# AgentCooper2002/AudioDiffuser

Hardware: AMD Instinct MI355X
Metric: audio samples/sec (16384-sample waveform, 50-step Heun) (higher is better)
Workload: dtype bf16; 1 GPU; BASELINE configs[1]: UNet1d 64 ch (c2), 16384-sample waveforms, KarrasSchedule N=50 heun, batch 64/GPU, random-init weights; global_batch=64, sampler=heun, num_steps=50, nfe=99, hipgraph=True, parallelism=batch-sharded x1, one all-gather

## Files before the change

audiodiffuser_amd/_lib.py:

```python
from __future__ import annotations

import ctypes as C
import os
from typing import Optional

from .config import UNet1dConfig

HERE = os.path.dirname(os.path.abspath(__file__))
LIB_PATH = os.environ.get("ADF_HIP_LIB") or os.path.join(HERE, "libadf_hip.so")
ADF_MAX_LAYERS = 12
DTYPE_F32, DTYPE_BF16, DTYPE_F32X3 = 0, 1, 2
FLAG_SEPARATE_GN_STATS = 1
SAMPLER_EDM, SAMPLER_EDM_ALPHA, SAMPLER_DPM_MULTISTEP, SAMPLER_DPM2, SAMPLER_ADPM2 = 0, 1, 2, 3, 4
SAMPLER_LMS, SAMPLER_DPM_SINGLESTEP, SAMPLER_DPM2M, SAMPLER_UNIPC, SAMPLER_ADPMPP2S = 5, 6, 7, 8, 9
SAMPLER_RF_EULER = 10


class AdfNetConfig(C.Structure):
    _fields_ = [
        ("channels", C.c_int32), ("num_filters", C.c_int32), ("window_length", C.c_int32), ("stride", C.c_int32),
        ("in_channels", C.c_int32), ("out_channels", C.c_int32),
        ("resnet_groups", C.c_int32), ("kernel_multiplier_downsample", C.c_int32),
        ("num_layers", C.c_int32),
        ("multipliers", C.c_int32 * (ADF_MAX_LAYERS + 1)),
# ... 116 lines not shown
    "adf_unet2d_create": (C.c_int, [C.POINTER(AdfUNet2dConfig), C.POINTER(C.c_void_p)]),
    "adf_dit_create": (C.c_int, [C.POINTER(AdfDitConfig), C.POINTER(C.c_void_p)]),
    "adf_set_image_shape": (C.c_int, [C.c_void_p, C.c_int, C.c_int]),
    "adf_set_dynamic_threshold": (C.c_int, [C.c_void_p, C.c_float]),
    "adf_set_preconditioning": (C.c_int, [C.c_void_p, C.c_int, C.c_double, C.c_double, C.c_double]),
    "adf_debug_coef_rows": (C.c_int, [C.c_void_p, C.c_void_p, C.c_int, C.POINTER(C.c_int), C.c_void_p]),
    "adf_destroy": (None, [C.c_void_p]),
    "adf_last_error": (C.c_char_p, [C.c_void_p]),
    "adf_num_weights": (C.c_int, [C.c_void_p]),
    "adf_weight_name": (C.c_char_p, [C.c_void_p, C.c_int]),
    "adf_weight_numel": (C.c_int64, [C.c_void_p, C.c_int]),
    "adf_load_weight": (C.c_int, [C.c_void_p, C.c_char_p, C.c_void_p, C.c_int64, C.c_void_p]),
    "adf_weights_missing": (C.c_int, [C.c_void_p]),
    "adf_set_condition": (C.c_int, [C.c_void_p, C.c_void_p, C.c_int, C.c_int, C.c_float, C.c_void_p]),
    "adf_net_forward": (C.c_int, [C.c_void_p, C.c_void_p, C.c_void_p, C.c_void_p, C.c_int, C.c_int, C.c_void_p]),
    "adf_denoise": (C.c_int, [C.c_void_p, C.c_void_p, C.c_void_p, C.c_float, C.c_float, C.c_void_p, C.c_int, C.c_int, C.c_void_p]),
    "adf_sampler_run": (C.c_int, [C.c_void_p, C.POINTER(AdfSamplerDesc), C.POINTER(C.c_float), C.c_int, C.c_void_p,
                                  C.c_void_p, C.c_int, C.c_void_p, C.c_int, C.c_int, C.c_void_p]),
    "adf_diffusion_loss": (C.c_int, [C.c_void_p, C.c_int, C.c_void_p, C.c_void_p, C.c_void_p, C.c_float, C.c_void_p, C.c_void_p, C.c_void_p,
                                     C.c_int, C.c_int, C.c_void_p]),
    "adf_loss_calls": (C.c_int64, [C.c_void_p]),
    "adf_sampler_nfe": (C.c_int, [C.POINTER(AdfSamplerDesc), C.POINTER(C.c_float), C.c_int]),
    "adf_sampler_run_table": (C.c_int, [C.c_void_p, C.POINTER(AdfTableDesc), C.POINTER(AdfTableStep), C.c_void_p, C.c_void_p, C.c_int, C.c_void_p,
                                        C.c_int, C.c_int, C.c_void_p]),
    "adf_sampler_table_nfe": (C.c_int, [C.POINTER(AdfTableDesc), C.POINTER(AdfTableStep)]),
    "adf_sampler_run_program": (C.c_int, [C.c_void_p, C.POINTER(AdfProgDesc), C.POINTER(AdfProgOp), C.c_void_p, C.c_void_p, C.c_int, C.c_int, C.c_void_p]),
    "adf_sampler_program_nfe": (C.c_int, [C.POINTER(AdfProgDesc), C.POINTER(AdfProgOp)]),
    "adf_debug_tap_shape": (C.c_int, [C.c_void_p, C.c_char_p, C.POINTER(C.c_int), C.POINTER(C.c_int)]),
    "adf_debug_tap_copy": (C.c_int, [C.c_void_p, C.c_char_p, C.c_void_p, C.c_void_p]),
    "adf_debug_tap_stats": (C.c_int, [C.c_void_p, C.c_char_p, C.c_void_p, C.POINTER(C.c_int), C.c_void_p]),
    "adf_debug_rb_block_plan": (C.c_int, [C.c_int] * 9 + [C.POINTER(C.c_int)] * 5),
    "adf_debug_up_tile_plan": (C.c_int, [C.c_int, C.c_int, C.c_int, C.c_int, C.c_int, C.POINTER(C.c_int), C.POINTER(C.c_int), C.POINTER(C.c_int),
                                         C.POINTER(C.c_int)]),
    "adf_debug_dyn_threshold": (C.c_int, [C.c_void_p, C.c_void_p, C.c_int, C.c_longlong, C.c_float, C.c_void_p]),
    "adf_debug_tap_count": (C.c_int, [C.c_void_p]),
    "adf_debug_tap_name": (C.c_char_p, [C.c_void_p, C.c_int]),
    "adf_device_bytes": (C.c_int64, [C.c_void_p]),
    "adf_bench_resblock": (C.c_int, [C.c_void_p, C.c_int, C.c_int, C.c_int, C.c_int, C.POINTER(C.c_float), C.POINTER(C.c_float),
                                     C.POINTER(C.c_double), C.POINTER(C.c_double), C.POINTER(C.c_double), C.POINTER(C.c_double),
                                     C.c_void_p]),
    "adf_bench_layer": (C.c_int, [C.c_void_p, C.c_int, C.c_int, C.c_int, C.c_int, C.c_int, C.POINTER(C.c_float), C.POINTER(C.c_double),
                                  C.POINTER(C.c_double), C.POINTER(C.c_int), C.c_void_p]),
    "adf_bench_wavenet_layer": (C.c_int, [C.c_void_p, C.c_int, C.c_int, C.c_int, C.c_int, C.POINTER(C.c_float), C.POINTER(C.c_double),
                                          C.POINTER(C.c_double), C.c_void_p]),
    "adf_bench_loss_kernels": (C.c_int, [C.c_void_p, C.c_int, C.c_int, C.c_longlong, C.c_int, C.POINTER(C.c_float), C.POINTER(C.c_float),
                                         C.POINTER(C.c_double), C.POINTER(C.c_double), C.c_void_p]),
    "adf_istft_create": (C.c_int, [C.POINTER(AdfIstftConfig), C.c_void_p, C.POINTER(C.c_void_p)]),
    "adf_istft_basis": (C.c_int, [C.POINTER(AdfIstftConfig), C.c_void_p, C.c_void_p, C.c_void_p]),
    "adf_istft_run": (C.c_int, [C.c_void_p, C.c_void_p, C.c_int, C.c_int, C.c_void_p, C.c_int64, C.c_void_p]),
    "adf_istft_destroy": (None, [C.c_void_p]),
    "adf_stft_create": (C.c_int, [C.POINTER(AdfIstftConfig), C.c_void_p, C.POINTER(C.c_void_p)]),
    "adf_stft_basis": (C.c_int, [C.POINTER(AdfIstftConfig), C.c_void_p, C.c_void_p]),
    "adf_stft_run": (C.c_int, [C.c_void_p, C.c_void_p, C.c_int, C.c_int64, C.c_void_p, C.c_int, C.c_void_p]),
    "adf_stft_destroy": (None, [C.c_void_p]),
}

_lib: Optional[C.CDLL] = None


def load_library() -> C.CDLL:
    global _lib
    if _lib is not None:
        return _lib
    if not os.path.exists(LIB_PATH):
        raise RuntimeError(
            f"{LIB_PATH} is missing: build it with `python -m audiodiffuser_amd.build` "
# ... 109 lines not shown
```

audiodiffuser_amd/csrc/adf_gemm.hip:

```cpp
#include "adf_gemm.h"
#include "adf_gemm_pp.h"
#include "adf_gemm_rb.h"
#include "adf_gemm_rbx3.h"
#include "adf_gemm_up.h"
#include "adf_kernels.h"
#include <cstdio>
#include <cstdlib>
#include <cstring>
#include <vector>


#ifdef ADF_RB_STAMP
namespace adf { __device__ unsigned long long adf_rb_stamps[8 * 16]; }
extern "C" int adf_debug_rb_stamps(unsigned long long* out) {
    return (int)hipMemcpyFromSymbol(out, HIP_SYMBOL(adf::adf_rb_stamps), sizeof(unsigned long long) * 8 * 16);
}
#endif

#ifdef ADF_RB_TL
namespace adf { __device__ unsigned adf_rb_tl[2 * 8 * 128]; }
extern "C" int adf_debug_rb_timeline(unsigned* out) {
    return (int)hipMemcpyFromSymbol(out, HIP_SYMBOL(adf::adf_rb_tl), sizeof(unsigned) * 2 * 8 * 128);
}
#endif
// ... 237 lines not shown
    if (a.n != a.n_pad || a.out_c != a.n || a.n_pad % kPpTN || a.n_pad > kPpMaxN) return false;
    if (!pow2(a.mrows / tm)) return false;
    if (a.res && a.nseg > 1) return false;
    int nb = a.res ? a.n / 64 : 0;
    for (int s = 0; s < a.nseg; ++s) {
        const GemmSeg& g = a.seg[s];
        if (g.stride != 1 || g.step != 1) return false;
        if (!((g.taps == 3 && g.off0 == -1) || (g.taps == 1 && g.off0 == 0))) return false;
        if (g.c0 % 64 || g.c1 % 64 || (g.ab && g.c0 + g.c1 > kPpMaxCin)) return false;
        if (s == 1 && (g.ab || g.act)) return false;
        nb += (g.c0 + g.c1) / 64;
    }
    return nb >= 2;
}

const void* pp_identity(int n, hipStream_t stream, const char** err) {
    static void* cache_dev[kMaxDevices][kPpMaxN / 64 + 1] = {};
    void** cache = cache_dev[current_device()];
    const int idx = n / 64;
    if (cache[idx]) return cache[idx];
    const size_t elems = (size_t)(n / 64 + kTapGroup) * n * 64;
    std::vector<uint16_t> hbuf(elems, 0);
    for (int r = 0; r < n; ++r) hbuf[((size_t)(r / 64) * n + r) * 64 + (r % 64)] = 0x3F80;
    void* d = nullptr;
    if (hipMalloc(&d, elems * 2) != hipSuccess) { *err = "conv_gemm_pp: hipMalloc(identity) failed"; return nullptr; }
    if (hipMemcpyAsync(d, hbuf.data(), elems * 2, hipMemcpyHostToDevice, stream) != hipSuccess || hipStreamSynchronize(stream) != hipSuccess) {
        *err = "conv_gemm_pp: identity upload failed";
        return nullptr;
    }
    cache[idx] = d;
    return d;
}

template <typename T, int MT, int NT>
const char* launch_ksplit(const GemmArgs& a, hipStream_t stream) {
    constexpr int lds = 4 * ks_wave_lds(MT, NT);
    constexpr int TM = 32 * MT, TN = 32 * NT;
    if (!raise_lds_limit<lds, conv_gemm_ksplit_kernel<T, MT, NT>>()) return "hipFuncSetAttribute(MaxDynamicSharedMemorySize, ksplit) failed";
    const int tiles_n = (a.n_pad + TN - 1) / TN;
    const long long tiles_m = a.flat ? ((long long)a.B * a.mrows + TM - 1) / TM : (long long)((a.mrows + TM - 1) / TM) * a.B;
    const long long blocks = tiles_m * tiles_n;
    if (blocks <= 0 || blocks > 0x7fffffffLL) return "conv_gemm_ksplit: bad grid";
    hipLaunchKernelGGL((conv_gemm_ksplit_kernel<T, MT, NT>), dim3((unsigned)blocks), dim3(256), lds, stream, a);
    return hipGetLastError() == hipSuccess ? nullptr : "conv_gemm_ksplit: launch failed";
}

template <typename T>
const char* dispatch(const GemmArgs& a, int tm, int tn, hipStream_t s) {
    if (tm == 128 && tn == 128) return launch_variant<T, 2, 2, 2, 2>(a, s);
    if (tm == 128 && tn == 64) return launch_variant<T, 2, 1, 2, 2>(a, s);
    if (tm == 128 && tn == 32) return launch_variant<T, 1, 1, 4, 1>(a, s);
    if (tm == 64 && tn == 128) return launch_variant<T, 1, 2, 2, 2>(a, s);
    if (tm == 64 && tn == 64) return launch_variant<T, 1, 1, 2, 2>(a, s);
    if (tm == 64 && tn == 32) return launch_variant<T, 1, 1, 2, 1>(a, s);
    if (tm == 32 && tn == 128) return launch_variant<T, 1, 1, 1, 4>(a, s);
    if (tm == 32 && tn == 64) return launch_variant<T, 1, 1, 1, 2>(a, s);
    return launch_variant<T, 1, 1, 1, 1>(a, s);
}

struct GemmSwitches {
    int trace = adf_route_switch("ADF_GEMM_TRACE", 0);
    int up = adf_route_switch("ADF_GEMM_UP", 1);
    int pp = adf_route_switch("ADF_GEMM_PP", 1);
    int ws = adf_route_switch("ADF_GEMM_WS", 1);
    long long rb_min_tiles = min_tiles_of(adf_route_switch("ADF_GEMM_RB", 1));
    long long rbx3_min_tiles = min_tiles_of(adf_route_switch("ADF_GEMM_RBX3", 1));
    int rb_zskip = adf_route_switch("ADF_RB_ZSKIP", 1);
    int gn_in_kernel = (int)adf_tuning("ADF_GEMM_GN", 1);
    int min_blocks = (int)adf_tuning("ADF_GEMM_MINBLOCKS", 512);
    int ksplit = (int)adf_tuning("ADF_GEMM_KSPLIT", 1);
    long long ksplit_rows = adf_tuning("ADF_GEMM_KSPLIT_ROWS", 4096);
    int ksplit_minit = (int)adf_tuning("ADF_GEMM_KSPLIT_MINIT", 4);
    long long ws_min_m = adf_tuning("ADF_GEMM_WS_MINM", 256);
    static long long min_tiles_of(int sw) { return sw == 0 ? -1 : (sw >= 2 ? 32 : 256); }
};
const GemmSwitches& switches() {
    static const GemmSwitches s;
    return s;
}

enum class Route { refused, up, ksplit, rbx3, rb, pp, ws, plain };
const char* const kRouteName[] = {"", "up", "ksplit", "rbx3", "rb", "pp", "ws", "plain"};

struct GemmPlan {
    Route route = Route::refused;
    const char* refusal = nullptr;
    int tm = 0, tn = 0;
    int flat = 0, seg_rows = 0;
    bool stats = false;
    bool stats_traced = false;
    bool gn_in_kernel = false;
    int up_cfg = 0;
    bool ident_seg = false;
};

bool rb_takes(const GemmArgs& a, bool x3, bool with_stats) {
    const long long min_tiles = x3 ? switches().rbx3_min_tiles : switches().rb_min_tiles;
    const RbForm& f = x3 ? kRbX3 : kRbBf16;
    RbTiles t;
    return min_tiles >= 0 && rb_shape_ok(a, f, with_stats) && rb_tiles(a, f, min_tiles, t);
// ... 163 lines not shown
    if (!p.stats) a.stats = nullptr;
    if (a.nseg > 1) a.seg[1].gn.gamma = nullptr;
    if (p.ident_seg) {
        const char* err = nullptr;
        const void* ident = pp_identity(a.n, stream, &err);
        if (!ident) return err;
        GemmSeg& g = a.seg[1];
        g = GemmSeg{};
        g.src0 = a.res; g.src1 = nullptr; g.c0 = a.n; g.c1 = 0; g.ab = nullptr; g.scale1 = 1.0f; g.act = 0;
        g.taps = 1; g.stride = 1; g.off0 = 0; g.step = 1; g.w = ident; g.nchunk = a.n / 64;
        a.nseg = 2;
        a.res = nullptr;
    }
    if (a.seg[0].gn.gamma && !p.gn_in_kernel) {
        const char* err = a.gn_ready ? nullptr : launch_gn_finalize(a.seg[0].gn, stream);
        a.seg[0].gn.gamma = nullptr;
        if (err) return err;
    }
    if (sw.trace) {
        fprintf(stderr, "[adf gemm] %-6s B=%d lin=%d mrows=%d n=%d/%d nseg=%d seg0(c=%d+%d taps=%d stride=%d off0=%d step=%d ab=%d act=%d)", kRouteName[(int)p.route], a.B,
                a.lin, a.mrows, a.n, a.n_pad, a.nseg, a.seg[0].c0, a.seg[0].c1, a.seg[0].taps, a.seg[0].stride, a.seg[0].off0, a.seg[0].step, a.seg[0].ab != nullptr,
                a.seg[0].act);
        if (a.nseg > 1) fprintf(stderr, " seg1(c=%d+%d taps=%d ab=%d)", a.seg[1].c0, a.seg[1].c1, a.seg[1].taps, a.seg[1].ab != nullptr);
        fprintf(stderr, " res=%d gelu=%d scatter=%d out=%dx%d stats=%d flat=%d tile=%dx%d\n", a.res != nullptr, a.gelu, a.scatter_f, a.out_rows, a.out_c, p.stats_traced,
                a.flat, p.tm, p.tn);
    }
    switch (p.route) {
    case Route::up:
        if (p.up_cfg == 1) return launch_up<256, 256, 4>(a, stream);
        if (p.up_cfg == 2) return launch_up<256, 128, 2>(a, stream);
        if (p.up_cfg == 3) return launch_up<128, 128, 2>(a, stream);
        return launch_up<128, 64, 2>(a, stream);
    case Route::ksplit:
        if (p.tm == 64) return dtype == 1 ? launch_ksplit<bf16_t, 2, 2>(a, stream) : (dtype == 2 ? launch_ksplit<f32x3_t, 2, 2>(a, stream) : launch_ksplit<float, 2, 2>(a, stream));
        return dtype == 1 ? launch_ksplit<bf16_t, 1, 1>(a, stream) : (dtype == 2 ? launch_ksplit<f32x3_t, 1, 1>(a, stream) : launch_ksplit<float, 1, 1>(a, stream));
    case Route::rbx3: return launch_rbx3(a, sw.rbx3_min_tiles, stream);
    case Route::rb: return launch_rb(a, sw.rb_min_tiles, sw.rb_zskip, stream);
    case Route::pp: return p.tm == 256 ? launch_pp<2>(a, stream) : launch_pp<1>(a, stream);
    case Route::ws:
        if (p.tn == 128) return dtype == 1 ? launch_ws_variant<bf16_t, 2, 2>(a, stream) : launch_ws_variant<float, 2, 2>(a, stream);
        return dtype == 1 ? launch_ws_variant<bf16_t, 1, 2>(a, stream) : launch_ws_variant<float, 1, 2>(a, stream);
    default: return dtype == 1 ? dispatch<bf16_t>(a, p.tm, p.tn, stream) : (dtype == 2 ? dispatch<f32x3_t>(a, p.tm, p.tn, stream) : dispatch<float>(a, p.tm, p.tn, stream));
    }
}

}

extern "C" int adf_debug_rb_block_plan(int K, int f, int C, int phase_c, int n, int B, int L, int min_tiles, int zskip, int* tile_rows, int* nh, int* nb3, int* nb2,
                                       int* phase2) {
    using namespace adf;
    if (B < 1 || L < 1 || C < 1 || f < 1 || (long long)B * L > 0x3fffffffLL) return 1;
    static const char dummy[16] = {};
    GemmArgs a;
    memset(&a, 0, sizeof(a));
    a.nseg = 1; a.B = B; a.lin = a.mrows = a.out_rows = L; a.n = a.n_pad = a.out_c = a.bias_mod = n;
    a.phase_c = phase_c;
    GemmSeg& g = a.seg[0];
    g.src0 = g.w = dummy;
    g.c0 = phase_c ? C : f * C;
    g.taps = 3; g.stride = 1; g.off0 = -1; g.step = 1;
    g.tap2_zero_c = phase_c ? 0 : folded_tap2_zero_from(K, f, C);
    RbTiles t;
    if (!rb_shape_ok(a, kRbBf16, false) || !rb_tiles(a, kRbBf16, min_tiles, t)) return 1;
    RbArgs r;
    rb_fill_args(a, kRbBf16, t, zskip, r);
    if (tile_rows) *tile_rows = t.tm;
    if (nh) *nh = t.nh;
    if (nb3) *nb3 = r.h.nb3;
    if (nb2) *nb2 = r.h.nb2;
    if (phase2) *phase2 = r.h.phase2;
    return 0;
}

extern "C" int adf_debug_up_tile_plan(int cin, int cout, int f, int B, int L, int* tile_rows, int* items, int* rounds, int* dead_rows) {
    using namespace adf;
    if (B < 1 || L < 1 || (long long)B * L > 0x3fffffffLL) return 1;
    UpTilePlan tp;
    if (cin == 256 && cout == 256 && f == 4) tp = up_tile_plan(B, L, UpCfg<256, 256, 4, 1>::WROWS, UpCfg<256, 256, 4, 1>::NPASS);
    else if (cin == 256 && cout == 128 && f == 2) tp = up_tile_plan(B, L, UpCfg<256, 128, 2, 1>::WROWS, UpCfg<256, 128, 2, 1>::NPASS);
    else if (cin == 128 && cout == 128 && f == 2) tp = up_tile_plan(B, L, UpCfg<128, 128, 2, 1>::WROWS, UpCfg<128, 128, 2, 1>::NPASS);
    else if (cin == 128 && cout == 64 && f == 2) tp = up_tile_plan(B, L, UpCfg<128, 64, 2, 1>::WROWS, UpCfg<128, 64, 2, 1>::NPASS);
    else return 1;
    if (tile_rows) *tile_rows = tp.tile_rows;
    if (items) *items = (int)tp.items;
    if (rounds) *rounds = (int)tp.rounds;
    if (dead_rows) *dead_rows = tp.dead_rows;
    return 0;
}
```

audiodiffuser_amd/csrc/adf_kernels.h:

```cpp
#pragma once
#include "adf_common.h"

namespace adf {

const char* launch_gn_stats(const void* x, int bf16, int B, int L, int C, int G, double* stats, hipStream_t s);

const char* launch_gn_finalize(const GnFinalizeArgs& a, hipStream_t s);

const char* launch_gn_apply(const void* s0, const void* s1, int c0, int c1, int L, int B, const float* ab, int act, void* out,
                            int bf16, hipStream_t s);

const char* launch_gn_norm_apply(const void* s0, const void* s1, const GnFinalizeArgs& a, int act, void* out, int bf16, hipStream_t s);

const char* launch_ln_rows(const void* x, void* y, int bf16, long long rows, int C, const float* gamma,
                           const float* beta, float eps, hipStream_t s);

const char* launch_attention(const void* qkv, void* out, int bf16, int B, int N, int C, int heads, hipStream_t s);
const char* launch_attention_x3(const void* qkv, void* out, int B, int N, int C, int heads, hipStream_t s);

const char* launch_upsample_nearest_pad(const void* x, void* out, int bf16, int B, int L, int C, int f, hipStream_t s);
const char* launch_to_in(const float* x, const float* w, void* out, int bf16, int B, int in_ch, int L, int nf,
                         int wl, int stride, int pad, const float* coef, int coef_bstride, hipStream_t s);

const char* launch_to_out(const void* h, const float* w, float* out, int dtype, int B, int out_ch, int Lh, int nf,
                          int wl, int stride, int pad, int mode, const float* x_noisy, const float* coef,
                          int coef_bstride, hipStream_t s);

enum { ADF_PRECOND_KIND_EDM = 0, ADF_PRECOND_KIND_VE = 1, ADF_PRECOND_KIND_VP = 2, ADF_PRECOND_KIND_V_EDM = 3, ADF_PRECOND_KIND_RF = 4, ADF_PRECOND_KIND_RF_EDM = 5 };
struct Precond {
    int kind = ADF_PRECOND_KIND_EDM;
    float sigma_data = 1.0f;
    float beta_min2 = 0.f, two_beta_d = 0.f, beta_min = 0.f, beta_d = 1.f, m_minus_1 = 0.f;
};
const char* launch_edm_coef(const float* sigmas_dev, float sigma_scalar, int nb, const Precond& pc, float* coef,
                            hipStream_t s);
const char* launch_edm_coef_list(const float* sigmas_host, int n, const Precond& pc, float* coef, hipStream_t s);

struct TimeEmbedArgs {
    const float* t; int t_stride; int nb; int ch;
    const float* fourier; const float* w1; const float* b1; const float* w2; const float* b2;
    float* temb;
};
const char* launch_time_embed(const TimeEmbedArgs& a, hipStream_t s);

const char* launch_film(const float* in, int in_dim, const float* w, int ldw, int w_col0, const float* bias, float* film, int nb,
                        int total, hipStream_t s);
const char* launch_class_embed(const long long* classes, int num_classes, int null_all, const float* emb, const float* null_emb,
                               const float* lnw, const float* lnb, const float* w1, const float* b1, const float* w2, const float* b2,
                               int ch, int cdim, float* out, int nrows, hipStream_t s);
const char* launch_cfg_combine(float* out, const float* x, const float* fc, const float* fn, const float* coef, int coef_bstride,
                               float scale, long long per_sample, long long n, int clampit, hipStream_t s);
const char* launch_dyn_threshold(float* x, int B, long long per_sample, float q, float* scale_scratch, hipStream_t s);

const char* launch_scale(float* out, const float* in, float s, long long n, hipStream_t st);
const char* launch_churn(float* x_hat, const float* x, const float* eps, float c, float s_noise, long long n, hipStream_t st);
// ... 35 lines not shown
```

audiodiffuser_amd/csrc/adf_kernels.hip:

```cpp
#include "adf_kernels.h"

namespace adf {

#define ADF_LAUNCH_CHECK(name) (hipGetLastError() == hipSuccess ? nullptr : name ": launch failed")

template <typename T>
__global__ void __launch_bounds__(256) gn_stats_kernel(const T* __restrict__ x, int L, int C, int G, int rows_per_block,
                                                       double* __restrict__ stats) {
    constexpr int EPC = Elem<T>::kPerChunk;
    extern __shared__ __attribute__((aligned(16))) char smem[];
    float* csum = (float*)smem;
    float* csq = csum + C;
    const int b = blockIdx.y;
    const int cpr = C / EPC;
    const int tid = threadIdx.x;
    for (int i = tid; i < 2 * C; i += 256) csum[i] = 0.f;
    __syncthreads();
    const int cc = tid % cpr, rsub = tid / cpr, rstep = 256 / cpr;
    const int r0 = blockIdx.x * rows_per_block;
    const int r1 = min(L, r0 + rows_per_block);
    float s[EPC], q[EPC];
#pragma unroll
    for (int e = 0; e < EPC; ++e) { s[e] = 0.f; q[e] = 0.f; }
    const T* base = x + (size_t)b * L * C + (size_t)cc * EPC;
// ... 814 lines not shown
        const int p0 = m0 * STRIDE - 4 + i * 4;
        float4 v = {0.f, 0.f, 0.f, 0.f};
        if (p0 >= 0 && p0 + 3 < L) v = *(const float4*)(xr + p0);
        else {
            if (p0 >= 0 && p0 < L) v.x = xr[p0];
            if (p0 + 1 >= 0 && p0 + 1 < L) v.y = xr[p0 + 1];
            if (p0 + 2 >= 0 && p0 + 2 < L) v.z = xr[p0 + 2];
            if (p0 + 3 >= 0 && p0 + 3 < L) v.w = xr[p0 + 3];
        }
        *(float4*)(xs + i * 4) = float4{cin * v.x, cin * v.y, cin * v.z, cin * v.w};
    }
    float wr[WL][EPC];
#pragma unroll
    for (int k = 0; k < WL; ++k)
#pragma unroll
        for (int e = 0; e < EPC; ++e) wr[k][e] = w[(size_t)(cc * EPC + e) * WL + k];
    __syncthreads();
    const int shift = 4 - pad;
#pragma unroll 4
    for (int ml = rsub; ml < ROWS && m0 + ml < Lo; ml += rpi) {
        float acc[EPC];
#pragma unroll
        for (int e = 0; e < EPC; ++e) acc[e] = 0.f;
#pragma unroll
        for (int k = 0; k < WL; ++k) {
            const float xv = xs[ml * STRIDE + k + shift];
#pragma unroll
            for (int e = 0; e < EPC; ++e) acc[e] = fmaf(wr[k][e], xv, acc[e]);
        }
        *(u32x4_t*)(out + ((size_t)b * Lo + m0 + ml) * nf + (size_t)cc * EPC) = pack16<T>(acc);
    }
}

const char* launch_to_in(const float* x, const float* w, void* out, int bf16, int B, int in_ch, int L, int nf,
                         int wl, int stride, int pad, const float* coef, int coef_bstride, hipStream_t s) {
    const int epc = bf16 ? 8 : 4;
    if (nf % epc) return "to_in: num_filters must be a multiple of a 16-byte chunk";
    if (L % stride) return "to_in: L % stride != 0";
    const int cpr_fast = nf / epc;
    if (in_ch == 1 && wl == 8 && stride == 2 && pad >= 0 && pad <= 4 && L % 4 == 0 && cpr_fast <= 256 && (cpr_fast & (cpr_fast - 1)) == 0) {
        const int Lo = L / stride;
        dim3 grid((unsigned)((Lo + 255) / 256), B);
        if (bf16) hipLaunchKernelGGL(to_in_rows_kernel<bf16_t>, grid, dim3(256), 0, s, x, w, (bf16_t*)out, L, nf, pad, coef, coef_bstride);
        else hipLaunchKernelGGL(to_in_rows_kernel<float>, grid, dim3(256), 0, s, x, w, (float*)out, L, nf, pad, coef, coef_bstride);
        return ADF_LAUNCH_CHECK("to_in_rows");
    }
    const size_t lds = (size_t)nf * in_ch * wl * sizeof(float);
    if (lds > 60000) return "to_in: weight tile too large for LDS";
    const long long work = (long long)(L / stride) * (nf / epc);
    dim3 grid((unsigned)((work + 255) / 256), B);
    if (bf16) hipLaunchKernelGGL(to_in_kernel<bf16_t>, grid, dim3(256), lds, s, x, w, (bf16_t*)out, in_ch, L, nf, wl, stride, pad, coef, coef_bstride);
    else hipLaunchKernelGGL(to_in_kernel<float>, grid, dim3(256), lds, s, x, w, (float*)out, in_ch, L, nf, wl, stride, pad, coef, coef_bstride);
    return ADF_LAUNCH_CHECK("to_in");
}

template <typename T>
__global__ void __launch_bounds__(256) to_out_kernel(const T* __restrict__ h, const float* __restrict__ w, float* __restrict__ out,
                                                     int out_ch, int Lh, int nf, int wl, int stride, int pad, int mode,
                                                     const float* __restrict__ x_noisy, const float* __restrict__ coef,
                                                     int coef_bstride) {
    constexpr int EPC = Elem<T>::kPerChunk;
    constexpr int R = 256;
    extern __shared__ __attribute__((aligned(16))) char smem[];
    const int halo = (wl + stride - 1) / stride;
    float* ws = (float*)smem;
    float* P = ws + nf * wl;
    const int b = blockIdx.y, oc = blockIdx.z;
    for (int i = threadIdx.x; i < nf * wl; i += 256) {
        const int k = i % wl, ci = i / wl;
        ws[i] = w[((size_t)ci * out_ch + oc) * wl + k];
    }
    __syncthreads();
    const int i0 = blockIdx.x * R - halo;
    const int nrows = R + 2 * halo;
// ... 111 lines not shown
        if (r < wl) {
#pragma unroll
            for (int e = 0; e < 16; ++e) {
                const int rr = t * 32 + (e & 3) + 8 * (e >> 2) + 4 * hh;
                const int ii = i0 + rr;
                if (rr < nrows) P[rr * wl + r] = (ii >= 0 && ii < Lh) ? acc[e] : 0.f;
            }
        }
    }
    __syncthreads();
    const int L = Lh * stride;
    const int l0 = blockIdx.x * R * stride;
    float c_skip = 0.f, c_out = 1.f;
    if (mode == 1) { c_skip = coef[(size_t)b * coef_bstride + 2]; c_out = coef[(size_t)b * coef_bstride + 3]; }
    for (int t = threadIdx.x; t < R * stride; t += 256) {
        const int l = l0 + t;
        if (l >= L) break;
        float acc = 0.f;
        const int k0 = (l + pad) % stride;
        for (int k = k0; k < wl; k += stride) {
            const int i = (l + pad - k) / stride;
            if (i >= 0 && i < Lh && (l + pad - k) >= 0) acc += P[(i - i0) * wl + k];
        }
        const size_t o = ((size_t)b * out_ch + oc) * L + l;
        float v = acc;
        if (mode == 1) {
            v = fmaf(c_skip, x_noisy[o], c_out * acc);
            v = fminf(fmaxf(v, -1.0f), 1.0f);
        }
        out[o] = v;
    }
}

__global__ void __launch_bounds__(256) to_out_x3_kernel(const float* __restrict__ h, const float* __restrict__ w, float* __restrict__ out,
                                                        int out_ch, int Lh, int nf, int wl, int stride, int pad, int mode,
                                                        const float* __restrict__ x_noisy, const float* __restrict__ coef,
                                                        int coef_bstride) {
    constexpr int R = 256;
    constexpr int MAXKS = 8;
    constexpr int PITCH = 272;
    extern __shared__ __attribute__((aligned(16))) char smem[];
    const int halo = (wl + stride - 1) / stride;
    float* P = (float*)smem;
    const int b = blockIdx.y, oc = blockIdx.z;
    const int lane = threadIdx.x & 63, wave = threadIdx.x >> 6;
    const int r = lane & 31, hh = lane >> 5;
    const int ksteps = nf / 16;
    to_bf16x8_t bh[MAXKS], bl[MAXKS];
#pragma unroll
    for (int ks = 0; ks < MAXKS; ++ks) {
        u32x4_t qh = u32x4_t{0u, 0u, 0u, 0u}, ql = qh;
        if (ks < ksteps && r < wl) {
            float f[8];
#pragma unroll
            for (int j = 0; j < 8; ++j) f[j] = w[((size_t)(16 * ks + 8 * hh + j) * out_ch + oc) * wl + r];
            u32x2_t h0, l0, h1, l1;
            split_bf16x4(f, h0, l0);
            split_bf16x4(f + 4, h1, l1);
            qh = u32x4_t{h0.x, h0.y, h1.x, h1.y};
            ql = u32x4_t{l0.x, l0.y, l1.x, l1.y};
        }
        bh[ks] = __builtin_bit_cast(to_bf16x8_t, qh);
        bl[ks] = __builtin_bit_cast(to_bf16x8_t, ql);
    }
    const int i0 = blockIdx.x * R - halo;
    const int nrows = R + 2 * halo;
// ... 45 lines not shown
    __syncthreads();
    const int L = Lh * stride;
    const int l0 = blockIdx.x * R * stride;
    float c_skip = 0.f, c_out = 1.f;
    if (mode == 1) { c_skip = coef[(size_t)b * coef_bstride + 2]; c_out = coef[(size_t)b * coef_bstride + 3]; }
    for (int t = threadIdx.x; t < R * stride; t += 256) {
        const int l = l0 + t;
        if (l >= L) break;
        float acc = 0.f;
        const int k0 = (l + pad) % stride;
        for (int k = k0; k < wl; k += stride) {
            const int i = (l + pad - k) / stride;
            if (i >= 0 && i < Lh && (l + pad - k) >= 0) acc += P[(i - i0) * wl + k];
        }
        const size_t o = ((size_t)b * out_ch + oc) * L + l;
        float v = acc;
        if (mode == 1) {
            v = fmaf(c_skip, x_noisy[o], c_out * acc);
            v = fminf(fmaxf(v, -1.0f), 1.0f);
        }
        out[o] = v;
    }
}

const char* launch_to_out(const void* h, const float* w, float* out, int dtype, int B, int out_ch, int Lh, int nf,
                          int wl, int stride, int pad, int mode, const float* x_noisy, const float* coef,
                          int coef_bstride, hipStream_t s) {
    const int bf16 = dtype == 1;
    const int epc = bf16 ? 8 : 4;
    if (nf % epc) return "to_out: num_filters must be a multiple of a 16-byte chunk";
    if (wl > 16) return "to_out: window_length > 16 unsupported";
    const int halo = (wl + stride - 1) / stride;
    dim3 grid(ceil_div(Lh, 256), B, out_ch);
    if (bf16 && nf % 16 == 0 && nf <= 128) {
        const size_t lds = (size_t)round_up(256 + 2 * halo, 32) * wl * sizeof(float) + 4 * 32 * 144;
        hipLaunchKernelGGL(to_out_mfma_kernel, grid, dim3(256), lds, s, (const bf16_t*)h, w, out, out_ch, Lh, nf, wl, stride, pad, mode, x_noisy, coef, coef_bstride);
        return ADF_LAUNCH_CHECK("to_out_mfma");
    }
    if (dtype == 2 && nf % 64 == 0 && nf <= 128) {
        const size_t lds = (size_t)round_up(256 + 2 * halo, 32) * wl * sizeof(float) + 4 * 32 * 272;
        hipLaunchKernelGGL(to_out_x3_kernel, grid, dim3(256), lds, s, (const float*)h, w, out, out_ch, Lh, nf, wl, stride, pad, mode, x_noisy, coef, coef_bstride);
        return ADF_LAUNCH_CHECK("to_out_x3");
    }
    const size_t lds = ((size_t)nf * wl + (size_t)(256 + 2 * halo) * wl) * sizeof(float);
    if (bf16) hipLaunchKernelGGL(to_out_kernel<bf16_t>, grid, dim3(256), lds, s, (const bf16_t*)h, w, out, out_ch, Lh, nf, wl, stride, pad, mode, x_noisy, coef, coef_bstride);
    else hipLaunchKernelGGL(to_out_kernel<float>, grid, dim3(256), lds, s, (const float*)h, w, out, out_ch, Lh, nf, wl, stride, pad, mode, x_noisy, coef, coef_bstride);
    return ADF_LAUNCH_CHECK("to_out");
}

__device__ __forceinline__ float precond_log(float x) { return (float)log((double)x); }
__device__ __forceinline__ float precond_exp(float x) { return (float)exp((double)x); }
__device__ __forceinline__ float precond_sqrt(float x) { return (float)sqrt((double)x); }
__device__ __forceinline__ float precond_div(float a, float b) { return (float)((double)a / (double)b); }
__device__ __forceinline__ float precond_mul(float a, float b) { return (float)((double)a * (double)b); }
__device__ __forceinline__ float precond_add(float a, float b) { return (float)((double)a + (double)b); }
__device__ __forceinline__ float precond_sigmoid(float x) { return precond_div(1.0f, precond_add(1.0f, precond_exp(-x))); }
__device__ __forceinline__ void precond_row(const Precond& pc, float s, float* __restrict__ row) {
    if (pc.kind == ADF_PRECOND_KIND_VE) {
        row[0] = 1.0f;
        row[1] = precond_log(precond_mul(0.5f, s));
        row[2] = 1.0f;
        row[3] = s;
    } else if (pc.kind == ADF_PRECOND_KIND_VP) {
        const float s2 = precond_mul(s, s);
        const float l = precond_log(precond_add(1.0f, s2));
        const float t = precond_div(precond_add(precond_sqrt(precond_add(pc.beta_min2, precond_mul(pc.two_beta_d, l))), -pc.beta_min), pc.beta_d);
        row[0] = precond_div(1.0f, precond_sqrt(precond_add(s2, 1.0f)));
        row[1] = precond_mul(pc.m_minus_1, t);
// ... 620 lines not shown
```

include/audiodiffuser_amd.h:

```cpp
#ifndef AUDIODIFFUSER_AMD_H
#define AUDIODIFFUSER_AMD_H

#include <stdint.h>

#ifdef __cplusplus
extern "C" {
#endif

#define ADF_ABI_VERSION 7
int adf_abi_version(void);

#define ADF_MAX_LAYERS 12

#define ADF_DTYPE_F32 0
#define ADF_DTYPE_BF16 1
#define ADF_DTYPE_F32X3 2

typedef struct adf_net_config {
    int32_t channels, num_filters, window_length, stride, in_channels, out_channels;
    int32_t resnet_groups, kernel_multiplier_downsample;
    int32_t num_layers;
    int32_t multipliers[ADF_MAX_LAYERS + 1];
    int32_t factors[ADF_MAX_LAYERS];
    int32_t num_blocks[ADF_MAX_LAYERS];
// ... 147 lines not shown
int adf_sampler_run_table(adf_handle* h, const adf_table_desc* desc, const adf_table_step* steps, const float* noise, const float* injected_noise,
                          int n_injected, float* out, int B, int L, void* stream);
int adf_sampler_table_nfe(const adf_table_desc* desc, const adf_table_step* steps);

#define ADF_PROG_EVAL 0
#define ADF_PROG_LIN 1
#define ADF_PROG_SLOTS 8
#define ADF_PROG_TERMS 5
typedef struct adf_prog_op {
    int32_t kind;
    int32_t dst;
    int32_t src;
    adf_table_eval eval;
    int32_t n_terms;
    int32_t slot[ADF_PROG_TERMS];
    float coef[ADF_PROG_TERMS];
    int32_t clamp;
} adf_prog_op;
typedef struct adf_prog_desc {
    int32_t num_ops;
    int32_t result_slot;
    float x0_scale;
    int32_t use_graph;
} adf_prog_desc;
int adf_sampler_run_program(adf_handle* h, const adf_prog_desc* desc, const adf_prog_op* ops, const float* noise, float* out, int B, int L, void* stream);
int adf_sampler_program_nfe(const adf_prog_desc* desc, const adf_prog_op* ops);

int adf_debug_tap_shape(adf_handle* h, const char* name, int* C, int* L);
int adf_debug_tap_copy(adf_handle* h, const char* name, float* out_fp32, void* stream);
int adf_debug_tap_stats(adf_handle* h, const char* name, double* out_host, int* groups, void* stream);
int adf_debug_up_tile_plan(int cin, int cout, int f, int B, int L, int* tile_rows, int* items, int* rounds, int* dead_rows);
int adf_debug_rb_block_plan(int K, int f, int C, int phase_c, int n, int B, int L, int min_tiles, int zskip, int* tile_rows, int* nh, int* nb3, int* nb2,
                            int* phase2);
int adf_debug_dyn_threshold(adf_handle* h, float* x_dev, int B, long long per_sample, float quantile, void* stream);
int adf_debug_coef_rows(adf_handle* h, float* out_dev, int max_rows, int* n_rows, void* stream);
int adf_debug_tap_count(adf_handle* h);
const char* adf_debug_tap_name(adf_handle* h, int index);

typedef struct adf_run_counters {
    int64_t sampler_runs;
    int64_t sampler_evals;
    int64_t graph_captures;
    int64_t graph_replays;
    int64_t denoise_calls;
    int64_t net_passes;
} adf_run_counters;
int adf_get_counters(const adf_handle* h, adf_run_counters* out);

int64_t adf_device_bytes(const adf_handle* h);

int adf_bench_resblock(adf_handle* h, int B, int L, int level, int iters, float* ms_block1, float* ms_block2,
                       double* algo_bytes_block1, double* algo_bytes_block2, double* flops_block1,
                       double* flops_block2, void* stream);
int adf_bench_layer(adf_handle* h, int B, int L, int level, int conv, int iters, float* ms, double* algo_bytes, double* flops,
                    int* copies, void* stream);

int adf_bench_wavenet_layer(adf_handle* h, int B, int T, int layer, int iters, float* ms, double* algo_bytes, double* flops, void* stream);

int adf_bench_loss_kernels(adf_handle* h, int rf, int B, long long N, int iters, float* ms_mix, float* ms_partial, double* bytes_mix,
                           double* bytes_partial, void* stream);

typedef struct adf_istft_config {
    int32_t n_fft, hop_length, center, normalized;
    double spec_abs_exponent, spec_factor;
} adf_istft_config;
typedef struct adf_istft_plan adf_istft_plan;
// ... 16 lines not shown
```

Measured before the change: 4.698 million audio-samples/s.

## Add persistent streaming to_in/to_out kernels and k-split zero-tap chunk skipping

Adds streaming versions of the input and output projection kernels. Each block now walks a run of several 256-row windows, double-buffering the waveform and hidden-state loads, and a run-length planner chooses the run so that the block count stays at or above 512 slots. This is meant to cut per-block setup costs such as weight loads and halo recomputation, and to overlap loads with compute. It also passes a zero-tap chunk boundary into the bf16 k-split GEMM so that padded zero channels of the third tap can be skipped. The cost is larger and more complex kernels with fewer blocks, which may lower parallelism.

```diff
diff --git a/audiodiffuser_amd/_lib.py b/audiodiffuser_amd/_lib.py
--- a/audiodiffuser_amd/_lib.py
+++ b/audiodiffuser_amd/_lib.py
@@ -172,6 +172,8 @@
     "adf_debug_rb_block_plan": (C.c_int, [C.c_int] * 9 + [C.POINTER(C.c_int)] * 5),
     "adf_debug_up_tile_plan": (C.c_int, [C.c_int, C.c_int, C.c_int, C.c_int, C.c_int, C.POINTER(C.c_int), C.POINTER(C.c_int), C.POINTER(C.c_int),
                                          C.POINTER(C.c_int)]),
+    "adf_debug_io_run_plan": (C.c_int, [C.c_int] * 3 + [C.POINTER(C.c_int)] * 4),
+    "adf_debug_ksplit_zero_chunks": (C.c_int, [C.c_int] * 4 + [C.POINTER(C.c_int)] * 2),
     "adf_debug_dyn_threshold": (C.c_int, [C.c_void_p, C.c_void_p, C.c_int, C.c_longlong, C.c_float, C.c_void_p]),
     "adf_debug_tap_count": (C.c_int, [C.c_void_p]),
     "adf_debug_tap_name": (C.c_char_p, [C.c_void_p, C.c_int]),
diff --git a/audiodiffuser_amd/csrc/adf_gemm.hip b/audiodiffuser_amd/csrc/adf_gemm.hip
--- a/audiodiffuser_amd/csrc/adf_gemm.hip
+++ b/audiodiffuser_amd/csrc/adf_gemm.hip
@@ -293,8 +293,15 @@
     return d;
 }
 
+int ksplit_zero_chunk(const GemmArgs& a, int zskip) {
+    const GemmSeg& g0 = a.seg[0];
+    return zskip && g0.taps == 3 && g0.tap2_zero_c > 0 && g0.tap2_zero_c % 64 == 0 && g0.tap2_zero_c < g0.c0 + g0.c1 ? g0.tap2_zero_c / 64 : 0;
+}
+
 template <typename T, int MT, int NT>
-const char* launch_ksplit(const GemmArgs& a, hipStream_t stream) {
+const char* launch_ksplit(const GemmArgs& a0, int zskip, hipStream_t stream) {
+    GemmArgs a = a0;
+    a.seg[0].tap2_zero_c = ksplit_zero_chunk(a0, zskip) * 64;
     constexpr int lds = 4 * ks_wave_lds(MT, NT);
     constexpr int TM = 32 * MT, TN = 32 * NT;
     if (!raise_lds_limit<lds, conv_gemm_ksplit_kernel<T, MT, NT>>()) return "hipFuncSetAttribute(MaxDynamicSharedMemorySize, ksplit) failed";
@@ -327,6 +334,7 @@
     long long rb_min_tiles = min_tiles_of(adf_route_switch("ADF_GEMM_RB", 1));
     long long rbx3_min_tiles = min_tiles_of(adf_route_switch("ADF_GEMM_RBX3", 1));
     int rb_zskip = adf_route_switch("ADF_RB_ZSKIP", 1);
+    int ks_zskip = adf_route_switch("ADF_KS_ZSKIP", 1);
     int gn_in_kernel = (int)adf_tuning("ADF_GEMM_GN", 1);
     int min_blocks = (int)adf_tuning("ADF_GEMM_MINBLOCKS", 512);
     int ksplit = (int)adf_tuning("ADF_GEMM_KSPLIT", 1);
@@ -556,8 +564,8 @@
         if (p.up_cfg == 3) return launch_up<128, 128, 2>(a, stream);
         return launch_up<128, 64, 2>(a, stream);
     case Route::ksplit:
-        if (p.tm == 64) return dtype == 1 ? launch_ksplit<bf16_t, 2, 2>(a, stream) : (dtype == 2 ? launch_ksplit<f32x3_t, 2, 2>(a, stream) : launch_ksplit<float, 2, 2>(a, stream));
-        return dtype == 1 ? launch_ksplit<bf16_t, 1, 1>(a, stream) : (dtype == 2 ? launch_ksplit<f32x3_t, 1, 1>(a, stream) : launch_ksplit<float, 1, 1>(a, stream));
+        if (p.tm == 64) return dtype == 1 ? launch_ksplit<bf16_t, 2, 2>(a, sw.ks_zskip, stream) : (dtype == 2 ? launch_ksplit<f32x3_t, 2, 2>(a, 0, stream) : launch_ksplit<float, 2, 2>(a, 0, stream));
+        return dtype == 1 ? launch_ksplit<bf16_t, 1, 1>(a, sw.ks_zskip, stream) : (dtype == 2 ? launch_ksplit<f32x3_t, 1, 1>(a, 0, stream) : launch_ksplit<float, 1, 1>(a, 0, stream));
     case Route::rbx3: return launch_rbx3(a, sw.rbx3_min_tiles, stream);
     case Route::rb: return launch_rb(a, sw.rb_min_tiles, sw.rb_zskip, stream);
     case Route::pp: return p.tm == 256 ? launch_pp<2>(a, stream) : launch_pp<1>(a, stream);
@@ -596,6 +604,31 @@
     return 0;
 }
 
+extern "C" int adf_debug_io_run_plan(int B, int rows, int sw, int* window, int* run, int* blocks_per_sample, int* blocks) {
+    using namespace adf;
+    if (B < 1 || rows < 1 || (long long)B * rows > 0x3fffffffLL) return 1;
+    const IoRunPlan p = io_run_plan(B, rows, sw);
+    if (window) *window = kIoWindow;
+    if (run) *run = p.run;
+    if (blocks_per_sample) *blocks_per_sample = p.blocks_per_sample;
+    if (blocks) *blocks = (int)p.blocks;
+    return 0;
+}
+
+extern "C" int adf_debug_ksplit_zero_chunks(int K, int f, int C, int zskip, int* nchunk, int* first_two_tap) {
+    using namespace adf;
+    if (K < 1 || f < 1 || C < 1 || (f * C) % 64 || (K - 1) / f + 1 != 3) return 1;
+    GemmArgs a;
+    memset(&a, 0, sizeof(a));
+    a.nseg = 1;
+    a.seg[0].c0 = f * C; a.seg[0].taps = 3;
+    a.seg[0].tap2_zero_c = folded_tap2_zero_from(K, f, C);
+    const int z = ksplit_zero_chunk(a, zskip);
+    if (nchunk) *nchunk = f * C / 64;
+    if (first_two_tap) *first_two_tap = z ? z : f * C / 64;
+    return 0;
+}
+
 extern "C" int adf_debug_up_tile_plan(int cin, int cout, int f, int B, int L, int* tile_rows, int* items, int* rounds, int* dead_rows) {
     using namespace adf;
     if (B < 1 || L < 1 || (long long)B * L > 0x3fffffffLL) return 1;
diff --git a/audiodiffuser_amd/csrc/adf_kernels.h b/audiodiffuser_amd/csrc/adf_kernels.h
--- a/audiodiffuser_amd/csrc/adf_kernels.h
+++ b/audiodiffuser_amd/csrc/adf_kernels.h
@@ -21,6 +21,22 @@
 const char* launch_upsample_nearest_pad(const void* x, void* out, int bf16, int B, int L, int C, int f, hipStream_t s);
 const char* launch_to_in(const float* x, const float* w, void* out, int bf16, int B, int in_ch, int L, int nf,
                          int wl, int stride, int pad, const float* coef, int coef_bstride, hipStream_t s);
+
+constexpr int kIoWindow = 256, kIoSlots = 512, kIoMaxWindows = 8;
+struct IoRunPlan { int run, blocks_per_sample; long long blocks, rounds; };
+inline IoRunPlan io_run_plan(int B, int rows, int sw = 1) {
+    const int slots = sw == 2 ? 1 : kIoSlots;
+    IoRunPlan best{};
+    for (int n = 1; n <= kIoMaxWindows; n *= 2) {
+        IoRunPlan c{};
+        c.run = kIoWindow * n;
+        c.blocks_per_sample = (rows + c.run - 1) / c.run;
+        c.blocks = (long long)B * c.blocks_per_sample;
+        c.rounds = (c.blocks + slots - 1) / slots;
+        if (n == 1 || c.blocks >= slots) best = c;
+    }
+    return best;
+}
 
 const char* launch_to_out(const void* h, const float* w, float* out, int dtype, int B, int out_ch, int Lh, int nf,
                           int wl, int stride, int pad, int mode, const float* x_noisy, const float* coef,
diff --git a/audiodiffuser_amd/csrc/adf_kernels.hip b/audiodiffuser_amd/csrc/adf_kernels.hip
--- a/audiodiffuser_amd/csrc/adf_kernels.hip
+++ b/audiodiffuser_amd/csrc/adf_kernels.hip
@@ -870,6 +870,71 @@
     }
 }
 
+template <typename T>
+__global__ void __launch_bounds__(256) to_in_stream_kernel(const float* __restrict__ x, const float* __restrict__ w, T* __restrict__ out, int L,
+                                                           int nf, int pad, int run, const float* __restrict__ coef, int coef_bstride) {
+    constexpr int EPC = Elem<T>::kPerChunk;
+    constexpr int WL = 8, STRIDE = 2, ROWS = kIoWindow;
+    constexpr int WIN = ROWS * STRIDE + 8;
+    static_assert(WIN / 4 <= 256, "one 16-byte waveform load per thread and window");
+    __shared__ __attribute__((aligned(16))) float xs[2][WIN];
+    const int b = blockIdx.y;
+    const int cpr = nf / EPC;
+    const int cc = threadIdx.x % cpr, rsub = threadIdx.x / cpr;
+    const int rpi = 256 / cpr;
+    const int Lo = L / STRIDE;
+    const int m_lo = blockIdx.x * run;
+    const int m_hi = min(m_lo + run, Lo);
+    const float cin = coef ? coef[(size_t)b * coef_bstride] : 1.0f;
+    const float* xr = x + (size_t)b * L;
+    auto load_window = [&](int m0) -> float4 {
+        float4 v = {0.f, 0.f, 0.f, 0.f};
+        if (threadIdx.x < WIN / 4) {
+            const int p0 = m0 * STRIDE - 4 + (int)threadIdx.x * 4;
+            if (p0 >= 0 && p0 + 3 < L) v = *(const float4*)(xr + p0);
+            else {
+                if (p0 >= 0 && p0 < L) v.x = xr[p0];
+                if (p0 + 1 >= 0 && p0 + 1 < L) v.y = xr[p0 + 1];
+                if (p0 + 2 >= 0 && p0 + 2 < L) v.z = xr[p0 + 2];
+                if (p0 + 3 >= 0 && p0 + 3 < L) v.w = xr[p0 + 3];
+            }
+        }
+        return v;
+    };
+    float4 nx = load_window(m_lo);
+    float wr[WL][EPC];
+#pragma unroll
+    for (int k = 0; k < WL; ++k)
+#pragma unroll
+        for (int e = 0; e < EPC; ++e) wr[k][e] = w[(size_t)(cc * EPC + e) * WL + k];
+    const int shift = 4 - pad;
+    int buf = 0;
+    for (int m0 = m_lo; m0 < m_hi; m0 += ROWS, buf ^= 1) {
+        float* const xw = xs[buf];
+        if (threadIdx.x < WIN / 4) *(float4*)(xw + threadIdx.x * 4) = float4{cin * nx.x, cin * nx.y, cin * nx.z, cin * nx.w};
+        __syncthreads();
+        if (m0 + ROWS < m_hi) nx = load_window(m0 + ROWS);
+#pragma unroll 4
+        for (int ml = rsub; ml < ROWS && m0 + ml < m_hi; ml += rpi) {
+            float acc[EPC];
+#pragma unroll
+            for (int e = 0; e < EPC; ++e) acc[e] = 0.f;
+#pragma unroll
+            for (int k = 0; k < WL; ++k) {
+                const float xv = xw[ml * STRIDE + k + shift];
+#pragma unroll
+                for (int e = 0; e < EPC; ++e) acc[e] = fmaf(wr[k][e], xv, acc[e]);
+            }
+            *(u32x4_t*)(out + ((size_t)b * Lo + m0 + ml) * nf + (size_t)cc * EPC) = pack16<T>(acc);
+        }
+    }
+}
+
+int io_stream_switch() {
+    static const int on = adf_route_switch("ADF_IO_STREAM", 1);
+    return on;
+}
+
 const char* launch_to_in(const float* x, const float* w, void* out, int bf16, int B, int in_ch, int L, int nf,
                          int wl, int stride, int pad, const float* coef, int coef_bstride, hipStream_t s) {
     const int epc = bf16 ? 8 : 4;
@@ -878,6 +943,13 @@
     const int cpr_fast = nf / epc;
     if (in_ch == 1 && wl == 8 && stride == 2 && pad >= 0 && pad <= 4 && L % 4 == 0 && cpr_fast <= 256 && (cpr_fast & (cpr_fast - 1)) == 0) {
         const int Lo = L / stride;
+        if (io_stream_switch()) {
+            const IoRunPlan p = io_run_plan(B, Lo, io_stream_switch());
+            dim3 grid((unsigned)p.blocks_per_sample, B);
+            if (bf16) hipLaunchKernelGGL(to_in_stream_kernel<bf16_t>, grid, dim3(256), 0, s, x, w, (bf16_t*)out, L, nf, pad, p.run, coef, coef_bstride);
+            else hipLaunchKernelGGL(to_in_stream_kernel<float>, grid, dim3(256), 0, s, x, w, (float*)out, L, nf, pad, p.run, coef, coef_bstride);
+            return ADF_LAUNCH_CHECK("to_in_stream");
+        }
         dim3 grid((unsigned)((Lo + 255) / 256), B);
         if (bf16) hipLaunchKernelGGL(to_in_rows_kernel<bf16_t>, grid, dim3(256), 0, s, x, w, (bf16_t*)out, L, nf, pad, coef, coef_bstride);
         else hipLaunchKernelGGL(to_in_rows_kernel<float>, grid, dim3(256), 0, s, x, w, (float*)out, L, nf, pad, coef, coef_bstride);
@@ -1055,6 +1127,117 @@
     }
 }
 
+__global__ void __launch_bounds__(256) to_out_stream_kernel(const bf16_t* __restrict__ h, const float* __restrict__ w, float* __restrict__ out,
+                                                            int out_ch, int Lh, int wl, int stride, int pad, int run, int mode,
+                                                            const float* __restrict__ x_noisy, const float* __restrict__ coef,
+                                                            int coef_bstride) {
+    constexpr int NF = 64, TRIP = 128, RING = 512;
+    extern __shared__ __attribute__((aligned(16))) char smem[];
+    const int halo = (wl + stride - 1) / stride;
+    float* P = (float*)smem;
+    const int b = blockIdx.y, oc = blockIdx.z;
+    const int tid = threadIdx.x, lane = tid & 63;
+    const int wave = __builtin_amdgcn_readfirstlane(tid >> 6);
+    const int r = lane & 31, hh = lane >> 5;
+    to_bf16x8_t bf[4];
+#pragma unroll
+    for (int ks = 0; ks < 4; ++ks) {
+        u32x4_t q = u32x4_t{0u, 0u, 0u, 0u};
+        if (r < wl) {
+            float f[8];
+#pragma unroll
+            for (int j = 0; j < 8; ++j) f[j] = w[((size_t)(16 * ks + 8 * hh + j) * out_ch + oc) * wl + r];
+            q = pack16<bf16_t>(f);
+        }
+        bf[ks] = __builtin_bit_cast(to_bf16x8_t, q);
+    }
+    char* const tl = (char*)(P + (size_t)RING * wl) + wave * (32 * 144);
+    const int i_lo = blockIdx.x * run, i_hi = min(i_lo + run, Lh);
+    const int rs = i_lo - halo;
+    const int nt = (i_hi - i_lo + 2 * halo + 31) / 32;
+    const int ns = (nt + 3) / 4;
+    const int L = Lh * stride;
+    const int l_lo = i_lo * stride, l_hi = i_hi * stride;
+    float c_skip = 0.f, c_out = 1.f;
+    if (mode == 1) { c_skip = coef[(size_t)b * coef_bstride + 2]; c_out = coef[(size_t)b * coef_bstride + 3]; }
+    const bf16_t* const hb = h + (size_t)b * Lh * NF + (lane & 7) * 8;
+    const float* const xnp = mode == 1 ? x_noisy + ((size_t)b * out_ch + oc) * L : w;
+    float* const ob = out + ((size_t)b * out_ch + oc) * L;
+
+    auto load_tile = [&](int t, u32x4_t (&rv)[4]) __attribute__((always_inline)) {
+#pragma unroll
+        for (int q = 0; q < 4; ++q) {
+            const int ii = rs + t * 32 + q * 8 + (lane >> 3);
+            const int icc = ii < 0 ? 0 : (ii >= Lh ? Lh - 1 : ii);
+            rv[q] = *(const u32x4_t*)(hb + (size_t)icc * NF);
+        }
+    };
+    auto first = [&](int s) __attribute__((always_inline)) -> int { return s == 0 ? l_lo : (rs + TRIP * s) * stride - pad; };
+    auto last = [&](int s) __attribute__((always_inline)) -> int { return min((rs + TRIP * (s + 1)) * stride - pad, l_hi); };
+    auto load_xn = [&](int s) __attribute__((always_inline)) -> float {
+        const int l = first(s) + tid;
+        return xnp[(mode == 1 && s < ns && l < last(s)) ? l : 0];
+    };
+    auto trip = [&](int s, u32x4_t (&cur)[4], const float& xn_use, float& xn_next) __attribute__((always_inline)) {
+        const int t = 4 * s + wave;
+        const bool live = t < nt;
+        if (live) {
+#pragma unroll
+            for (int q = 0; q < 4; ++q) *(u32x4_t*)(tl + (q * 8 + (lane >> 3)) * 144 + (lane & 7) * 16) = cur[q];
+        }
+        __builtin_amdgcn_wave_barrier();
+        xn_next = load_xn(s + 1);
+        load_tile(t + 8, cur);
+        if (live) {
+            to_f32x16_t acc;
+#pragma unroll
+            for (int e = 0; e < 16; ++e) acc[e] = 0.f;
+#pragma unroll
+            for (int ks = 0; ks < 4; ++ks) {
+                const to_bf16x8_t af = *(const to_bf16x8_t*)(tl + r * 144 + (ks * 2 + hh) * 16);
+                acc = __builtin_amdgcn_mfma_f32_32x32x16_bf16(af, bf[ks], acc, 0, 0, 0);
+            }
+            __builtin_amdgcn_wave_barrier();
+            if (r < wl) {
+#pragma unroll
+                for (int e = 0; e < 16; ++e) {
+                    const int rr = t * 32 + (e & 3) + 8 * (e >> 2) + 4 * hh;
+                    const int ii = rs + rr;
+                    P[(rr & (RING - 1)) * wl + r] = (ii >= 0 && ii < Lh) ? acc[e] : 0.f;
+                }
+            }
+        }
+        __syncthreads();
+        const int l = first(s) + tid;
+        if (l < last(s)) {
+            float acc = 0.f;
+            const int k0 = (l + pad) % stride;
+            for (int k = k0; k < wl; k += stride) {
+                const int i = (l + pad - k) / stride;
+                if (i >= 0 && i < Lh && (l + pad - k) >= 0) acc += P[((i - rs) & (RING - 1)) * wl + k];
+            }
+            float v = acc;
+            if (mode == 1) {
+                v = fmaf(c_skip, xn_use, c_out * acc);
+                v = fminf(fmaxf(v, -1.0f), 1.0f);
+            }
+            ob[l] = v;
+        }
+    };
+    u32x4_t rva[4], rvb[4];
+    float xa, xb = 0.f;
+    load_tile(wave, rva);
+    __builtin_amdgcn_sched_barrier(0);
+    xa = load_xn(0);
+    __builtin_amdgcn_sched_barrier(0);
+    load_tile(4 + wave, rvb);
+    __builtin_amdgcn_sched_barrier(0);
+    for (int s = 0; s < ns; s += 2) {
+        trip(s, rva, xa, xb);
+        trip(s + 1, rvb, xb, xa);
+    }
+}
+
 __global__ void __launch_bounds__(256) to_out_x3_kernel(const float* __restrict__ h, const float* __restrict__ w, float* __restrict__ out,
                                                         int out_ch, int Lh, int nf, int wl, int stride, int pad, int mode,
                                                         const float* __restrict__ x_noisy, const float* __restrict__ coef,
@@ -1166,8 +1349,15 @@
     if (wl > 16) return "to_out: window_length > 16 unsupported";
     const int halo = (wl + stride - 1) / stride;
     dim3 grid(ceil_div(Lh, 256), B, out_ch);
+    if (bf16 && nf == 64 && stride <= 2 && pad >= 0 && pad <= halo * stride && io_stream_switch()) {
+        const IoRunPlan p = io_run_plan(B * out_ch, Lh, io_stream_switch());
+        const size_t lds = (size_t)512 * wl * sizeof(float) + 4 * 32 * 144;
+        hipLaunchKernelGGL(to_out_stream_kernel, dim3(p.blocks_per_sample, B, out_ch), dim3(256), lds, s, (const bf16_t*)h, w, out, out_ch, Lh, wl, stride, pad, p.run, mode,
+                           x_noisy, coef, coef_bstride);
+        return ADF_LAUNCH_CHECK("to_out_stream");
+    }
     if (bf16 && nf % 16 == 0 && nf <= 128) {
-        const size_t lds = (size_t)round_up(256 + 2 * halo, 32) * wl * sizeof(float) + 4 * 32 * 144;
+        const size_t lds =(size_t)round_up(256 + 2 * halo, 32) * wl * sizeof(float) + 4 * 32 * 144;
         hipLaunchKernelGGL(to_out_mfma_kernel, grid, dim3(256), lds, s, (const bf16_t*)h, w, out, out_ch, Lh, nf, wl, stride, pad, mode, x_noisy, coef, coef_bstride);
         return ADF_LAUNCH_CHECK("to_out_mfma");
     }
diff --git a/include/audiodiffuser_amd.h b/include/audiodiffuser_amd.h
--- a/include/audiodiffuser_amd.h
+++ b/include/audiodiffuser_amd.h
@@ -203,6 +203,8 @@
 int adf_debug_up_tile_plan(int cin, int cout, int f, int B, int L, int* tile_rows, int* items, int* rounds, int* dead_rows);
 int adf_debug_rb_block_plan(int K, int f, int C, int phase_c, int n, int B, int L, int min_tiles, int zskip, int* tile_rows, int* nh, int* nb3, int* nb2,
                             int* phase2);
+int adf_debug_io_run_plan(int B, int rows, int sw, int* window, int* run, int* blocks_per_sample, int* blocks);
+int adf_debug_ksplit_zero_chunks(int K, int f, int C, int zskip, int* nchunk, int* first_two_tap);
 int adf_debug_dyn_threshold(adf_handle* h, float* x_dev, int B, long long per_sample, float quantile, void* stream);
 int adf_debug_coef_rows(adf_handle* h, float* out_dev, int max_rows, int* n_rows, void* stream);
 int adf_debug_tap_count(adf_handle* h);
```

After: 4.718 million audio-samples/s (median of 6 runs). Within noise of the previous version (+0.4%).
